# baudm/parseq

Hardware: NVIDIA H100
Metric: images/sec PARSeq-S 32x128 AR+1refine (higher is better)
Workload: dtype bf16

## Files before the change

### include/parseq_b200.h

```cpp
#ifndef PARSEQ_B200_H_
#define PARSEQ_B200_H_

#include <stdint.h>

#ifdef __cplusplus
extern "C" {
#endif

typedef struct parseq_engine parseq_engine;
typedef void* parseq_stream_t;

typedef enum parseq_status {
  PARSEQ_OK = 0,
  PARSEQ_ERR_INVALID_ARG = -1,
  PARSEQ_ERR_UNSUPPORTED = -2,
  PARSEQ_ERR_CUDA = -3,
  PARSEQ_ERR_STATE = -4,
  PARSEQ_ERR_NO_DEVICE = -5
} parseq_status;

typedef struct parseq_config {
  int32_t img_h, img_w;
  int32_t patch_h, patch_w;
  int32_t embed_dim;
// ... 65 lines not shown
int64_t parseq_kernel_launches(const parseq_engine* e);
int parseq_bench_tma_stream(void* buf, int64_t bytes, int cluster, int ctas, int nboxes, int nslot, int mode, void* sink,
                            parseq_stream_t stream);
int64_t parseq_debug_int(parseq_engine* e, const char* name);
int parseq_set_option(parseq_engine* e, const char* name, int64_t value);
int parseq_get_timing(parseq_engine* e, int category, double* ms, double* flops, int64_t* count);
int parseq_get_ar_profile(parseq_engine* e, uint64_t* out512);
const char* parseq_last_error(void);
const char* parseq_version(void);

int parseq_gemm_bf16(const void* A, int64_t lda, const void* W, int64_t ldw, const float* bias,
                     int M, int N, int K, int mode, float alpha, const float* resid, int64_t ldr,
                     int resid_mod, void* out, int64_t ldo, parseq_stream_t stream);
int parseq_gemm_ln_bf16(const void* A, int64_t lda, const void* W, int64_t ldw, const float* bias,
                        int M, int D, int K, float* x_inout, const float* gamma, const float* beta,
                        float eps, void* xn_bf16, parseq_stream_t stream);
int parseq_mlp_ln_bf16(const void* xn, const void* W1, const float* b1, const void* W2, const float* b2,
                       int M, int D, float* x_inout, const float* gamma, const float* beta, float eps,
                       void* xn_out_bf16, parseq_stream_t stream);
int parseq_layernorm_bf16(const float* x, const float* gamma, const float* beta, float eps, int M,
                          int D, void* y_bf16, float* y_f32_or_null, parseq_stream_t stream);
int parseq_enc_attention(const void* qkv_bf16, int B, int T, int D, int heads, void* out_bf16,
                         parseq_stream_t stream);

#ifdef __cplusplus
}
#endif
#endif
```

### parseq_b200/build.py

```python
from __future__ import annotations

import os
import shutil
import subprocess

PKG = os.path.dirname(os.path.abspath(__file__))
CSRC = os.path.join(PKG, "csrc")
LIB_DIR = os.path.join(PKG, "lib")
LIB_PATH = os.path.join(LIB_DIR, "libparseq_b200.so")
SOURCES = ["engine.cu"]
HEADERS = ["ptx.cuh", "gemm.cuh", "kernels.cuh", "dec_ar.cuh", "dec_ar2.cuh", "gemm_ln.cuh", "mlp_ln.cuh", "attn_wgmma.cuh", "crops.cuh", os.path.join("..", "..", "include", "parseq_b200.h")]

NVCC_FLAGS = [
    "-gencode", "arch=compute_90a,code=sm_90a", "-lineinfo", "-O3", "-std=c++17",
    "-Xcompiler", "-fPIC", "-shared",
]


def _nvcc() -> str:
    for cand in (os.environ.get("NVCC"), shutil.which("nvcc"), "/usr/local/cuda/bin/nvcc"):
        if cand and os.path.exists(cand):
            return cand
    raise RuntimeError("nvcc not found")


def needs_build() -> bool:
    if not os.path.exists(LIB_PATH):
        return True
    t = os.path.getmtime(LIB_PATH)
    deps = [os.path.join(CSRC, s) for s in SOURCES + HEADERS]
    return any(os.path.getmtime(d) > t for d in deps)


def build(force: bool = False, verbose: bool = False) -> str:
# ... 26 lines not shown
```

### parseq_b200/csrc/engine.cu

```cuda
#include <cuda.h>
#include <cuda_runtime.h>

#include <cmath>
#include <cstdio>
#include <cstdlib>
#include <cstring>
#include <map>
#include <mutex>
#include <set>
#include <string>
#include <type_traits>
#include <vector>

#include "../../include/parseq_b200.h"
#include "gemm.cuh"
#include "kernels.cuh"
#include "dec_ar.cuh"
#include "dec_ar2.cuh"
#include "gemm_ln.cuh"
#include "mlp_ln.cuh"
#include "attn_wgmma.cuh"
#include "crops.cuh"

namespace {

constexpr int kMaxHeadClasses = 16384;
constexpr int kMaxLabelLength = 63;

thread_local std::string g_last_error;

int fail(int code, const std::string& msg) {
  g_last_error = msg;
  return code;
}
#define PQ_CUDA(expr)                                                                              \
  do {                                                                                             \
    cudaError_t _e = (expr);                                                                       \
    if (_e != cudaSuccess)                                                                         \
      return fail(PARSEQ_ERR_CUDA, std::string(#expr) + " -> " + cudaGetErrorString(_e));          \
  } while (0)
#define PQ_TRY(expr)                 \
  do {                               \
    int _r = (expr);                 \
    if (_r != PARSEQ_OK) return _r;  \
// ... 187 lines not shown
}
template <int D, int MT, int CS, bool WIDE, int IDP>
int ar2_attr() {
  PQ_TRY(set_smem(ar2_kernel<D, MT, CS, false, WIDE, IDP>(), pq::dec_ar2_smem_bytes<D, MT, CS, IDP>()));
  if constexpr (MT == 1 && CS == 8 && D / 64 <= CS)
    PQ_TRY(set_smem(ar2_kernel<D, MT, CS, true, WIDE, IDP>(), pq::dec_ar2_smem_bytes<D, MT, CS, IDP>()));
  return PARSEQ_OK;
}
template <bool WIDE, int IDP>
int ar2_set_attributes() {
  PQ_TRY((ar2_attr<192, 1, 8, WIDE, IDP>())); PQ_TRY((ar2_attr<192, 2, 8, WIDE, IDP>())); PQ_TRY((ar2_attr<384, 1, 8, WIDE, IDP>()));
  PQ_TRY((ar2_attr<384, 2, 8, WIDE, IDP>())); PQ_TRY((ar2_attr<768, 1, 8, WIDE, IDP>()));
  PQ_TRY((ar2_attr<192, 1, 6, WIDE, IDP>())); PQ_TRY((ar2_attr<192, 2, 6, WIDE, IDP>())); PQ_TRY((ar2_attr<384, 1, 6, WIDE, IDP>()));
  PQ_TRY((ar2_attr<384, 2, 6, WIDE, IDP>())); PQ_TRY((ar2_attr<768, 1, 6, WIDE, IDP>()));
  return PARSEQ_OK;
}

template <int D, int MODE>
int gemm_ln_attr() { return set_smem(pq::gemm_ln_fused_kernel<D, MODE>, pq::GemmLnCfg<D, MODE>::kSmemBytes); }
template <int D, int CG>
int mlp_ln_attr() { return set_smem(pq::mlp_ln_fused_kernel<D, CG>, pq::MlpLnCfg<D, CG>::kSmemBytes); }
template <int NK>
int attn_wgmma_attr() { return set_smem(pq::enc_attention_wgmma_kernel<NK>, pq::atw_smem_bytes<NK>()); }
template <int EPI, int STORE>
int gemm_attr() { return set_smem(pq::gemm_bf16_wgmma_kernel<EPI, STORE>, pq::GemmCfg::smem_bytes<STORE != pq::ST_REG>()); }
constexpr int kTmaBenchSmem = 12 * pq::A2_SLOT + 1024 + 256;

int init_kernel_attributes() {
  PQ_TRY(set_smem(pq::dec_ar_kernel<192, 1>, pq::dec_ar_smem_bytes<192>()));
  PQ_TRY(set_smem(pq::dec_ar_kernel<192, 2>, pq::dec_ar_smem_bytes<192>()));
  PQ_TRY(set_smem(pq::dec_ar_kernel<384, 1>, pq::dec_ar_smem_bytes<384>()));
  PQ_TRY(set_smem(pq::dec_ar_kernel<384, 2>, pq::dec_ar_smem_bytes<384>()));
  PQ_TRY(set_smem(pq::dec_ar_kernel<768, 1>, pq::dec_ar_smem_bytes<768>()));
  PQ_TRY(set_smem(pq::dec_ar_kernel<768, 2>, pq::dec_ar_smem_bytes<768>()));
  PQ_TRY((ar2_set_attributes<false, 32>()));
  PQ_TRY((ar2_set_attributes<true, 32>()));
  PQ_TRY((ar2_set_attributes<false, 64>()));
  PQ_TRY((ar2_set_attributes<true, 64>()));
  PQ_TRY(set_smem(pq::dec_ln_head_argmax_kernel<192>, 120 * 1024));
  PQ_TRY(set_smem(pq::dec_ln_head_argmax_kernel<384>, 160 * 1024));
  PQ_TRY(set_smem(pq::dec_ln_head_argmax_kernel<768>, 226 * 1024));
  PQ_TRY((gemm_ln_attr<192, 0>())); PQ_TRY((gemm_ln_attr<384, 0>())); PQ_TRY((gemm_ln_attr<192, 1>()));
  PQ_TRY((gemm_ln_attr<384, 1>())); PQ_TRY((gemm_ln_attr<384, 2>()));
  PQ_TRY((mlp_ln_attr<192, 1>())); PQ_TRY((mlp_ln_attr<384, 1>())); PQ_TRY((mlp_ln_attr<192, 2>())); PQ_TRY((mlp_ln_attr<384, 2>()));
  PQ_TRY((attn_wgmma_attr<128>())); PQ_TRY((attn_wgmma_attr<256>()));
  PQ_TRY((gemm_attr<pq::EPI_F32, pq::ST_REG>()));
  PQ_TRY((gemm_attr<pq::EPI_F32_RESID, pq::ST_REG>()));
  PQ_TRY((gemm_attr<pq::EPI_BF16, pq::ST_REG>()));
  PQ_TRY((gemm_attr<pq::EPI_BF16, pq::ST_TMA_2D>()));
  PQ_TRY((gemm_attr<pq::EPI_BF16, pq::ST_TMA_3D>()));
  PQ_TRY((gemm_attr<pq::EPI_GELU_BF16, pq::ST_REG>()));
  PQ_TRY((gemm_attr<pq::EPI_GELU_BF16, pq::ST_TMA_2D>()));
  PQ_TRY(set_smem(pq::tma_stream_bench_kernel, kTmaBenchSmem));
  int dev = 0, optin = 0;
  PQ_CUDA(cudaGetDevice(&dev));
  PQ_CUDA(cudaDeviceGetAttribute(&optin, cudaDevAttrMaxSharedMemoryPerBlockOptin, dev));
  PQ_TRY(set_smem(pq::crop_resize_bicubic_kernel, static_cast<size_t>(optin)));
  return PARSEQ_OK;
}

int ensure_kernel_attributes() {
  static std::mutex mu;
  static std::set<int> done;
  int dev = 0;
  PQ_CUDA(cudaGetDevice(&dev));
  std::lock_guard<std::mutex> lock(mu);
  if (done.count(dev) != 0) return PARSEQ_OK;
  PQ_TRY(init_kernel_attributes());
// ... 133 lines not shown
    case 192: return launch_k(lo, pq::layernorm_kernel<192>, dim3(grid), dim3(256), 0, st, x, g, b, eps, M, yb, y32, add, add_mod, xw);
    case 384: return launch_k(lo, pq::layernorm_kernel<384>, dim3(grid), dim3(256), 0, st, x, g, b, eps, M, yb, y32, add, add_mod, xw);
    case 768: return launch_k(lo, pq::layernorm_kernel<768>, dim3(grid), dim3(256), 0, st, x, g, b, eps, M, yb, y32, add, add_mod, xw);
    default: return fail(PARSEQ_ERR_UNSUPPORTED, "layernorm: embed_dim must be 192, 384 or 768");
  }
}

int enc_attention_launch(const LaunchOpts& lo, const void* qkv, int B, int T, int D, int heads, void* out, cudaStream_t st) {
  if (D != heads * pq::ATT_DH) return fail(PARSEQ_ERR_UNSUPPORTED, "encoder attention kernels cover head_dim=64");
  if (lo.attn_impl == 1 && T <= 256) {
    const dim3 grid(static_cast<unsigned>(B * heads), static_cast<unsigned>((T + 127) / 128));
    const __nv_bfloat16* q = reinterpret_cast<const __nv_bfloat16*>(qkv);
    __nv_bfloat16* o = reinterpret_cast<__nv_bfloat16*>(out);
    if (T <= 128)
      return launch_k(lo, pq::enc_attention_wgmma_kernel<128>, grid, dim3(pq::ATW_THREADS), pq::atw_smem_bytes<128>(), st, q, o, T, D, heads);
    return launch_k(lo, pq::enc_attention_wgmma_kernel<256>, grid, dim3(pq::ATW_THREADS), pq::atw_smem_bytes<256>(), st, q, o, T, D, heads);
  }
  if (T != pq::ATT_T) {
    return launch_k(lo, pq::enc_attention_any_kernel, dim3(B * heads, (T + pq::ATT_T - 1) / pq::ATT_T), dim3(256), 0, st,
                    reinterpret_cast<const __nv_bfloat16*>(qkv), reinterpret_cast<__nv_bfloat16*>(out), T, D, heads);
  }
  return launch_k(lo, pq::enc_attention_kernel, dim3(B * heads), dim3(256), 0, st,
                  reinterpret_cast<const __nv_bfloat16*>(qkv), reinterpret_cast<__nv_bfloat16*>(out), D, heads);
}

struct Slot {
  std::string key;
  std::string pub;
  long long numel;
  bool bf16;
  void* dev;
  bool set;
};

}

struct parseq_engine {
  parseq_config cfg;
  int D, T, Kp, Me, Md, L, V, C, gh, gw, dh_dec;
  int ids_ld = 32;
  int arch = 0, Tp = 0;
  std::map<std::string, int> pub_index;
  float* vt_rows = nullptr;
  int chunk;
  std::vector<Slot> slots;
  std::map<std::string, int> index;
// ... 237 lines not shown
  }
  if (e->arch == 0) {
    PQ_TRY(gemm(e, e->a_pe, e->Kp, e->w("encoder.patch_embed.proj.weight"), e->Kp,
                e->wf("encoder.patch_embed.proj.bias"), M, D, e->Kp, pq::EPI_F32, 1.0f, e->wf("encoder.pos_embed"), D, T,
                e->x, D, st));
  } else {
    float* tmp = reinterpret_cast<float*>(e->hid);
    PQ_TRY(gemm(e, e->a_pe, e->Kp, e->w("encoder.patch_embed.proj.weight"), e->Kp,
                e->wf("encoder.patch_embed.proj.bias"), B * e->Tp, D, e->Kp, pq::EPI_F32, 1.0f,
                e->wf("encoder.pos_embed") + D, D, e->Tp, tmp, D, st));
    TimedScope ts(e, st, CAT_MISC, 0.0);
    const long long total = 1ll * M * (D / 4);
    const int grid = static_cast<int>(std::min<long long>((total + 255) / 256, 132ll * 16));
    PQ_TRY(launch_k(e->lo, pq::cls_assemble_kernel, dim3(grid), dim3(256), 0, st, reinterpret_cast<const float4*>(tmp),
                    reinterpret_cast<const float4*>(e->wf("encoder.cls_token")),
                    reinterpret_cast<const float4*>(e->wf("encoder.pos_embed")), reinterpret_cast<float4*>(e->x), B, e->Tp,
                    D / 4));
  }
  const int Mr = (regime_batch > B ? regime_batch : B) * T;
  const bool big = (Mr + pq::GEMM_BLOCK_M - 1) / pq::GEMM_BLOCK_M >= 2 * e->lo.sm_count || (e->fuse_ln & 4);
  const bool fuse_proj = (e->fuse_ln & 1) && gemm_ln_supported(D) && big;
  const bool fuse_fc2 = (e->fuse_ln & 2) && gemm_ln_supported(D) && big;
  const bool fuse_mlp = e->fuse_mlp && fuse_fc2 && e->Me == 4 * D;
  bool final_done = false;
  for (int i = 0; i < e->cfg.enc_depth; ++i) {
    const std::string p = "encoder.blocks." + std::to_string(i) + ".";
    const bool last = (i == e->cfg.enc_depth - 1);
    if (!(fuse_fc2 && i > 0)) PQ_TRY(layernorm(e, e->x, p + "norm1", 1e-6f, M, e->xn, nullptr, st));
    PQ_TRY(gemm(e, e->xn, D, e->w(p + "attn.qkv.weight"), D, e->wf(p + "attn.qkv.bias"), M, 3 * D, D, pq::EPI_BF16,
                1.0f, nullptr, 0, 0, e->qkv, 3 * D, st));
    {
      TimedScope ts(e, st, CAT_ENC_ATTN, 4.0 * B * T * T * D);
      PQ_TRY(enc_attention_launch(e->lo, e->qkv, B, T, D, e->cfg.enc_num_heads, e->att, st));
    }
    if (fuse_proj) {
      PQ_TRY(gemm_ln(e, e->att, D, p + "attn.proj", M, D, e->x, p + "norm2", 1e-6f, e->xn, st));
    } else {
      PQ_TRY(gemm(e, e->att, D, e->w(p + "attn.proj.weight"), D, e->wf(p + "attn.proj.bias"), M, D, D, pq::EPI_F32, 1.0f,
                  e->x, D, 0, e->x, D, st));
      PQ_TRY(layernorm(e, e->x, p + "norm2", 1e-6f, M, e->xn, nullptr, st));
    }
    if (fuse_mlp && (!last || (final_norm && memory32 == nullptr))) {
      if (!last) {
        PQ_TRY(mlp_ln(e, e->xn, p, M, e->x, "encoder.blocks." + std::to_string(i + 1) + ".norm1", 1e-6f, e->xn, st));
      } else {
        PQ_TRY(mlp_ln(e, e->xn, p, M, e->x, "encoder.norm", 1e-6f, mem_out, st));
        final_done = true;
      }
      continue;
    }
    PQ_TRY(gemm(e, e->xn, D, e->w(p + "mlp.fc1.weight"), D, e->wf(p + "mlp.fc1.bias"), M, e->Me, D, pq::EPI_GELU_BF16,
                1.0f, nullptr, 0, 0, e->hid, e->Me, st));
    if (fuse_fc2 && !last) {
      PQ_TRY(gemm_ln(e, e->hid, e->Me, p + "mlp.fc2", M, e->Me, e->x, "encoder.blocks." + std::to_string(i + 1) + ".norm1",
// ... 1346 lines not shown
}
int parseq_gemm_ln_bf16(const void* A, int64_t lda, const void* W, int64_t ldw, const float* bias, int M, int D, int K,
                         float* x_inout, const float* gamma, const float* beta, float eps, void* xn_bf16,
                         parseq_stream_t stream) {
  PQ_TRY(ensure_kernel_attributes());
  return gemm_ln_launch(g_default_opts, A, lda, W, ldw, bias, M, D, K, x_inout, gamma, beta, eps, xn_bf16, reinterpret_cast<cudaStream_t>(stream));
}
int parseq_mlp_ln_bf16(const void* xn, const void* W1, const float* b1, const void* W2, const float* b2, int M, int D,
                       float* x_inout, const float* gamma, const float* beta, float eps, void* xn_out_bf16, parseq_stream_t stream) {
  PQ_TRY(ensure_kernel_attributes());
  return mlp_ln_launch(g_default_opts, xn, W1, b1, W2, b2, M, D, x_inout, gamma, beta, eps, xn_out_bf16,
                       reinterpret_cast<cudaStream_t>(stream));
}
int parseq_layernorm_bf16(const float* x, const float* gamma, const float* beta, float eps, int M, int D, void* y_bf16,
                          float* y_f32_or_null, parseq_stream_t stream) {
  PQ_TRY(ensure_kernel_attributes());
  return layernorm_launch(g_default_opts, x, gamma, beta, eps, M, D, y_bf16, y_f32_or_null, reinterpret_cast<cudaStream_t>(stream));
}
int parseq_enc_attention(const void* qkv_bf16, int B, int T, int D, int heads, void* out_bf16, parseq_stream_t stream) {
  PQ_TRY(ensure_kernel_attributes());
  PQ_TRY(ensure_sm_count(g_default_opts));
  return enc_attention_launch(g_default_opts, qkv_bf16, B, T, D, heads, out_bf16, reinterpret_cast<cudaStream_t>(stream));
}

}
```

### parseq_b200/csrc/kernels.cuh

```cuda
#pragma once
#include "ptx.cuh"

namespace pq {

__global__ void im2col_patch_kernel(const float* __restrict__ img, __nv_bfloat16* __restrict__ out, int B, int H,
                                    int W, int ph, int pw, int gh, int gw) {
  grid_dep_launch();
  grid_dep_wait();
  const long long total = static_cast<long long>(B) * gh * gw * 3 * ph;
  const int Kp = 3 * ph * pw;
  for (long long i = blockIdx.x * static_cast<long long>(blockDim.x) + threadIdx.x; i < total;
       i += static_cast<long long>(gridDim.x) * blockDim.x) {
    long long t = i;
    const int c = static_cast<int>(t % gw); t /= gw;
    const int ch = static_cast<int>(t % 3); t /= 3;
    const int dy = static_cast<int>(t % ph); t /= ph;
    const int r = static_cast<int>(t % gh); t /= gh;
    const int b = static_cast<int>(t);
    const float* src = img + ((static_cast<long long>(b) * 3 + ch) * H + (r * ph + dy)) * W + c * pw;
    __nv_bfloat16* dst = out + (static_cast<long long>(b) * gh * gw + r * gw + c) * Kp + ch * ph * pw + dy * pw;
    if (pw == 8 && ((reinterpret_cast<uintptr_t>(src) & 15u) == 0) && ((reinterpret_cast<uintptr_t>(dst) & 15u) == 0)) {
      const float4 a = __ldg(reinterpret_cast<const float4*>(src));
      const float4 d = __ldg(reinterpret_cast<const float4*>(src) + 1);
      uint4 q;
// ... 72 lines not shown
    q += a * a + b * b;
  }
#pragma unroll
  for (int o = 16; o > 0; o >>= 1) q += __shfl_xor_sync(0xffffffffu, q, o);
  const float rstd = 1.0f / sqrtf(q * (1.0f / D) + eps);
  const float2* g2 = reinterpret_cast<const float2*>(gamma);
  const float2* b2 = reinterpret_cast<const float2*>(beta);
  uint32_t* yr = reinterpret_cast<uint32_t*>(y + static_cast<long long>(row) * D);
#pragma unroll
  for (int i = 0; i < NV; ++i) {
    const float2 g = __ldg(g2 + i * 32 + lane), b = __ldg(b2 + i * 32 + lane);
    const float o0 = (v[i].x - mean) * rstd * g.x + b.x;
    const float o1 = (v[i].y - mean) * rstd * g.y + b.y;
    yr[i * 32 + lane] = pack_bf16(o0, o1);
    if (y32 != nullptr) reinterpret_cast<float2*>(y32 + static_cast<long long>(row) * D)[i * 32 + lane] = make_float2(o0, o1);
  }
}

constexpr int ATT_T = 128;
constexpr int ATT_DH = 64;
__device__ __forceinline__ uint32_t att_swz(int r, int c) {
  return static_cast<uint32_t>(r * ATT_DH + ((((c >> 3) ^ (r & 7)) << 3) | (c & 7)));
}
__global__ void __launch_bounds__(256, 2) enc_attention_kernel(const __nv_bfloat16* __restrict__ qkv,
                                                            __nv_bfloat16* __restrict__ out, int D, int heads) {
  grid_dep_launch();
  grid_dep_wait();
  __shared__ __align__(128) __nv_bfloat16 sQ[ATT_T * ATT_DH];
  __shared__ __align__(128) __nv_bfloat16 sK[ATT_T * ATT_DH];
  __shared__ __align__(128) __nv_bfloat16 sV[ATT_T * ATT_DH];
  const int b = blockIdx.x / heads, h = blockIdx.x % heads;
  const int tid = threadIdx.x, warp = tid >> 5, lane = tid & 31;
  const long long ld = 3ll * D;
  const __nv_bfloat16* base = qkv + static_cast<long long>(b) * ATT_T * ld + h * ATT_DH;
  for (int i = tid; i < 3 * ATT_T * 8; i += 256) {
    const int m = i / (ATT_T * 8);
    const int r = (i / 8) % ATT_T;
    const int ck = i % 8;
    const __nv_bfloat16* src = base + static_cast<long long>(r) * ld + m * D + ck * 8;
    __nv_bfloat16* dstm = (m == 0) ? sQ : (m == 1) ? sK : sV;
    cp_async_16(smem_u32(dstm + att_swz(r, ck * 8)), src);
  }
  cp_async_wait_all();
  __syncthreads();

  const int r0 = warp * 16;
  uint32_t qf[4][4];
#pragma unroll
  for (int kt = 0; kt < 4; ++kt) {
    const int row = r0 + (lane & 7) + ((lane >> 3) & 1) * 8;
    const int col = kt * 16 + (lane >> 4) * 8;
    ldmatrix_x4(smem_u32(sQ + att_swz(row, col)), qf[kt][0], qf[kt][1], qf[kt][2], qf[kt][3]);
  }
  float sacc[16][4];
#pragma unroll
  for (int nt = 0; nt < 16; ++nt) { sacc[nt][0] = sacc[nt][1] = sacc[nt][2] = sacc[nt][3] = 0.f; }
#pragma unroll
  for (int kt = 0; kt < 4; ++kt) {
#pragma unroll
    for (int np = 0; np < 8; ++np) {
      const int key = np * 16 + (lane & 7) + (lane >> 4) * 8;
      const int col = kt * 16 + ((lane >> 3) & 1) * 8;
      uint32_t b0, b1, b2, b3;
      ldmatrix_x4(smem_u32(sK + att_swz(key, col)), b0, b1, b2, b3);
      mma_bf16_16816(sacc[2 * np], qf[kt][0], qf[kt][1], qf[kt][2], qf[kt][3], b0, b1);
      mma_bf16_16816(sacc[2 * np + 1], qf[kt][0], qf[kt][1], qf[kt][2], qf[kt][3], b2, b3);
    }
  }
  float mx0 = -INFINITY, mx1 = -INFINITY;
#pragma unroll
  for (int nt = 0; nt < 16; ++nt) {
    mx0 = fmaxf(mx0, fmaxf(sacc[nt][0], sacc[nt][1]));
    mx1 = fmaxf(mx1, fmaxf(sacc[nt][2], sacc[nt][3]));
  }
  mx0 = fmaxf(mx0, __shfl_xor_sync(0xffffffffu, mx0, 1));
  mx0 = fmaxf(mx0, __shfl_xor_sync(0xffffffffu, mx0, 2));
  mx1 = fmaxf(mx1, __shfl_xor_sync(0xffffffffu, mx1, 1));
  mx1 = fmaxf(mx1, __shfl_xor_sync(0xffffffffu, mx1, 2));
  constexpr float kScaleLog2 = 0.125f * 1.4426950408889634f;
  float sum0 = 0.f, sum1 = 0.f;
#pragma unroll
  for (int nt = 0; nt < 16; ++nt) {
    sacc[nt][0] = exp2f((sacc[nt][0] - mx0) * kScaleLog2);
    sacc[nt][1] = exp2f((sacc[nt][1] - mx0) * kScaleLog2);
    sacc[nt][2] = exp2f((sacc[nt][2] - mx1) * kScaleLog2);
    sacc[nt][3] = exp2f((sacc[nt][3] - mx1) * kScaleLog2);
    sum0 += sacc[nt][0] + sacc[nt][1];
    sum1 += sacc[nt][2] + sacc[nt][3];
  }
  sum0 += __shfl_xor_sync(0xffffffffu, sum0, 1);
  sum0 += __shfl_xor_sync(0xffffffffu, sum0, 2);
  sum1 += __shfl_xor_sync(0xffffffffu, sum1, 1);
  sum1 += __shfl_xor_sync(0xffffffffu, sum1, 2);
  float oacc[8][4];
#pragma unroll
  for (int nt = 0; nt < 8; ++nt) { oacc[nt][0] = oacc[nt][1] = oacc[nt][2] = oacc[nt][3] = 0.f; }
#pragma unroll
  for (int kk = 0; kk < 8; ++kk) {
    const uint32_t a0 = pack_bf16(sacc[2 * kk][0], sacc[2 * kk][1]);
    const uint32_t a1 = pack_bf16(sacc[2 * kk][2], sacc[2 * kk][3]);
    const uint32_t a2 = pack_bf16(sacc[2 * kk + 1][0], sacc[2 * kk + 1][1]);
    const uint32_t a3 = pack_bf16(sacc[2 * kk + 1][2], sacc[2 * kk + 1][3]);
#pragma unroll
    for (int np = 0; np < 4; ++np) {
      const int key = kk * 16 + (lane & 7) + ((lane >> 3) & 1) * 8;
      const int col = np * 16 + (lane >> 4) * 8;
      uint32_t b0, b1, b2, b3;
      ldmatrix_x4_trans(smem_u32(sV + att_swz(key, col)), b0, b1, b2, b3);
      mma_bf16_16816(oacc[2 * np], a0, a1, a2, a3, b0, b1);
      mma_bf16_16816(oacc[2 * np + 1], a0, a1, a2, a3, b2, b3);
    }
  }
  const float inv0 = 1.0f / sum0, inv1 = 1.0f / sum1;
  const int g = lane >> 2, t = lane & 3;
  __syncwarp();
#pragma unroll
  for (int nt = 0; nt < 8; ++nt) {
    const int col = nt * 8 + 2 * t;
    *reinterpret_cast<uint32_t*>(sQ + att_swz(r0 + g, col)) = pack_bf16(oacc[nt][0] * inv0, oacc[nt][1] * inv0);
    *reinterpret_cast<uint32_t*>(sQ + att_swz(r0 + g + 8, col)) = pack_bf16(oacc[nt][2] * inv1, oacc[nt][3] * inv1);
  }
  __syncwarp();
  __nv_bfloat16* obase = out + static_cast<long long>(b) * ATT_T * D + h * ATT_DH;
#pragma unroll
  for (int i = 0; i < 4; ++i) {
    const int idx = i * 32 + lane;
    const int r = r0 + (idx >> 3), ck = idx & 7;
    const uint4 val = *reinterpret_cast<const uint4*>(sQ + att_swz(r, ck * 8));
    *reinterpret_cast<uint4*>(obase + static_cast<long long>(r) * D + ck * 8) = val;
  }
}

__global__ void __launch_bounds__(256, 2) enc_attention_any_kernel(const __nv_bfloat16* __restrict__ qkv,
                                                                   __nv_bfloat16* __restrict__ out, int T, int D,
                                                                   int heads) {
  grid_dep_launch();
  grid_dep_wait();
  __shared__ __align__(128) __nv_bfloat16 sQ[ATT_T * ATT_DH];
  __shared__ __align__(128) __nv_bfloat16 sK[ATT_T * ATT_DH];
  __shared__ __align__(128) __nv_bfloat16 sV[ATT_T * ATT_DH];
  const int b = blockIdx.x / heads, h = blockIdx.x % heads;
  const int q0 = blockIdx.y * ATT_T;
  const int nkb = (T + ATT_T - 1) / ATT_T;
  const int tid = threadIdx.x, warp = tid >> 5, lane = tid & 31;
  const long long ld = 3ll * D;
  const __nv_bfloat16* base = qkv + static_cast<long long>(b) * T * ld + h * ATT_DH;
  auto load_tile = [&](__nv_bfloat16* dst, int mat, int row0, int nrows) {
    for (int i = tid; i < nrows * 8; i += 256) {
      const int r = i >> 3, ck = i & 7;
      int row = row0 + r;
      if (row >= T) row = T - 1;
      cp_async_16(smem_u32(dst + att_swz(r, ck * 8)), base + static_cast<long long>(row) * ld + mat * D + ck * 8);
    }
// ... 658 lines not shown
```

### parseq_b200/engine.py

```python
from __future__ import annotations

import ctypes as C
import os
from typing import Dict, Optional

from .build import LIB_PATH

_lib = None


class ParseqConfigC(C.Structure):
    _fields_ = [(n, C.c_int32) for n in (
        "img_h", "img_w", "patch_h", "patch_w", "embed_dim", "enc_num_heads", "enc_mlp_ratio", "enc_depth",
        "dec_num_heads", "dec_mlp_ratio", "dec_depth", "max_label_length", "num_tokens", "max_batch", "device", "arch")]


class ForwardArgsC(C.Structure):
    _fields_ = [("batch", C.c_int32), ("max_length", C.c_int32), ("decode_ar", C.c_int32),
                ("refine_iters", C.c_int32), ("forced_ids", C.c_void_p), ("forced_refine", C.c_void_p)]


class CropsC(C.Structure):
    _fields_ = [("data", C.c_void_p), ("data_bytes", C.c_int64), ("offsets", C.c_void_p), ("sizes", C.c_void_p),
                ("rotation", C.c_int32)]


EXPORTS = [
    "parseq_create", "parseq_destroy", "parseq_set_weight", "parseq_num_weights", "parseq_weight_key",
    "parseq_finalize", "parseq_forward", "parseq_forward_host", "parseq_forward_u8", "parseq_forward_host_u8",
    "parseq_resize_crops", "parseq_forward_crops", "parseq_forward_host_crops",
    "parseq_postprocess", "parseq_encode", "parseq_decode", "parseq_decode_ex", "parseq_head", "parseq_text_embed", "parseq_kernel_launches", "parseq_debug_int", "parseq_bench_tma_stream",
    "parseq_set_option", "parseq_get_timing", "parseq_get_ar_profile", "parseq_last_error", "parseq_version", "parseq_gemm_bf16", "parseq_gemm_ln_bf16", "parseq_mlp_ln_bf16", "parseq_layernorm_bf16",
    "parseq_enc_attention",
]


def load_library(path: Optional[str] = None):
    global _lib
    if _lib is not None and path is None:
        return _lib
    p = path or os.environ.get("PARSEQ_B200_LIB", LIB_PATH)
    if not os.path.exists(p):
        raise RuntimeError(f"{p} not found: build it with `python -m parseq_b200.build` "
                           "(there is no CPU / PyTorch fallback)")
    lib = C.CDLL(p)
    lib.parseq_last_error.restype = C.c_char_p
    lib.parseq_version.restype = C.c_char_p
    lib.parseq_weight_key.restype = C.c_char_p
    lib.parseq_weight_key.argtypes = [C.c_void_p, C.c_int, C.POINTER(C.c_int64)]
    lib.parseq_bench_tma_stream.argtypes = [C.c_void_p, C.c_int64, C.c_int, C.c_int, C.c_int, C.c_int, C.c_int, C.c_void_p, C.c_void_p]
    lib.parseq_debug_int.restype = C.c_int64
    lib.parseq_debug_int.argtypes = [C.c_void_p, C.c_char_p]
    lib.parseq_kernel_launches.restype = C.c_int64
    lib.parseq_kernel_launches.argtypes = [C.c_void_p]
    lib.parseq_create.argtypes = [C.POINTER(ParseqConfigC), C.POINTER(C.c_void_p)]
    lib.parseq_destroy.argtypes = [C.c_void_p]
# ... 12 lines not shown
    lib.parseq_forward_host_crops.argtypes = lib.parseq_forward_crops.argtypes
    lib.parseq_postprocess.argtypes = [C.c_void_p, C.c_int32, C.c_int32, C.c_int32, C.c_int32, C.c_void_p, C.c_void_p,
                                       C.c_void_p, C.c_void_p]
    lib.parseq_encode.argtypes = [C.c_void_p, C.c_int32, C.c_void_p, C.c_void_p, C.c_void_p]
    lib.parseq_decode.argtypes = [C.c_void_p, C.c_int32, C.c_int32, C.c_int32, C.c_void_p, C.c_void_p, C.c_void_p, C.c_void_p,
                                  C.c_void_p, C.c_void_p, C.c_void_p]
    lib.parseq_decode_ex.argtypes = [C.c_void_p, C.c_int32, C.c_int32, C.c_int32, C.c_void_p, C.c_void_p, C.c_void_p, C.c_void_p,
                                     C.c_void_p, C.c_void_p, C.c_void_p, C.c_void_p]
    lib.parseq_head.argtypes = [C.c_void_p, C.c_int32, C.c_void_p, C.c_void_p, C.c_void_p]
    lib.parseq_text_embed.argtypes = [C.c_void_p, C.c_int32, C.c_void_p, C.c_void_p, C.c_void_p]
    lib.parseq_set_option.argtypes = [C.c_void_p, C.c_char_p, C.c_int64]
    lib.parseq_get_timing.argtypes = [C.c_void_p, C.c_int, C.POINTER(C.c_double), C.POINTER(C.c_double),
                                      C.POINTER(C.c_int64)]
    lib.parseq_gemm_bf16.argtypes = [C.c_void_p, C.c_int64, C.c_void_p, C.c_int64, C.c_void_p, C.c_int, C.c_int,
                                     C.c_int, C.c_int, C.c_float, C.c_void_p, C.c_int64, C.c_int, C.c_void_p,
                                     C.c_int64, C.c_void_p]
    lib.parseq_gemm_ln_bf16.argtypes = [C.c_void_p, C.c_int64, C.c_void_p, C.c_int64, C.c_void_p, C.c_int, C.c_int, C.c_int,
                                        C.c_void_p, C.c_void_p, C.c_void_p, C.c_float, C.c_void_p, C.c_void_p]
    lib.parseq_mlp_ln_bf16.argtypes = [C.c_void_p, C.c_void_p, C.c_void_p, C.c_void_p, C.c_void_p, C.c_int, C.c_int, C.c_void_p,
                                       C.c_void_p, C.c_void_p, C.c_float, C.c_void_p, C.c_void_p]
    lib.parseq_layernorm_bf16.argtypes = [C.c_void_p, C.c_void_p, C.c_void_p, C.c_float, C.c_int, C.c_int,
                                          C.c_void_p, C.c_void_p, C.c_void_p]
    lib.parseq_enc_attention.argtypes = [C.c_void_p, C.c_int, C.c_int, C.c_int, C.c_int, C.c_void_p, C.c_void_p]
    if path is None:
        _lib = lib
    return lib


class EngineError(RuntimeError):
    pass


def check(lib, rc: int):
    if rc != 0:
        raise EngineError(f"parseq_b200 error {rc}: {lib.parseq_last_error().decode()}")


class Engine:

    def __init__(self, cfg, device: int = 0, max_batch: int = 0):
        self.lib = load_library()
        self.cfg = cfg
        c = ParseqConfigC(cfg.img_size[0], cfg.img_size[1], cfg.patch_size[0], cfg.patch_size[1], cfg.embed_dim,
                          cfg.enc_num_heads, cfg.enc_mlp_ratio, cfg.enc_depth, cfg.dec_num_heads, cfg.dec_mlp_ratio,
                          cfg.dec_depth, cfg.max_label_length, cfg.num_tokens, max_batch, device,
                          1 if getattr(cfg, "arch", "parseq") == "vitstr" else 0)
# ... 118 lines not shown
```

Before: 38900.

## Fuse encoder QKV projection GEMM with attention in a persistent warp-specialized kernel

Adds a persistent kernel that, for each (batch, head) item, computes the Q/K/V projection for a 128-token tile with TMA-fed wgmma and writes the results straight into swizzled shared memory. It then runs the existing 128x128 attention tile on that data, so the QKV activation never round-trips through global memory and one launch is removed per layer. The attention body is factored into a shared device function. In exchange, the activation tile is re-read once per head, and occupancy is one 384-thread CTA per SM with a producer warp group.

```diff
diff --git a/include/parseq_b200.h b/include/parseq_b200.h
--- a/include/parseq_b200.h
+++ b/include/parseq_b200.h
@@ -111,6 +111,8 @@
                           int D, void* y_bf16, float* y_f32_or_null, parseq_stream_t stream);
 int parseq_enc_attention(const void* qkv_bf16, int B, int T, int D, int heads, void* out_bf16,
                          parseq_stream_t stream);
+int parseq_qkv_attention_bf16(const void* xn_bf16, const void* W_qkv, const float* b_qkv, int B, int T, int D,
+                              int heads, void* out_bf16, parseq_stream_t stream);
 
 #ifdef __cplusplus
 }
diff --git a/parseq_b200/build.py b/parseq_b200/build.py
--- a/parseq_b200/build.py
+++ b/parseq_b200/build.py
@@ -9,7 +9,7 @@
 LIB_DIR = os.path.join(PKG, "lib")
 LIB_PATH = os.path.join(LIB_DIR, "libparseq_b200.so")
 SOURCES = ["engine.cu"]
-HEADERS = ["ptx.cuh", "gemm.cuh", "kernels.cuh", "dec_ar.cuh", "dec_ar2.cuh", "gemm_ln.cuh", "mlp_ln.cuh", "attn_wgmma.cuh", "crops.cuh", os.path.join("..", "..", "include", "parseq_b200.h")]
+HEADERS = ["ptx.cuh", "gemm.cuh", "kernels.cuh", "dec_ar.cuh", "dec_ar2.cuh", "gemm_ln.cuh", "mlp_ln.cuh", "attn_wgmma.cuh", "qkv_attn.cuh", "crops.cuh", os.path.join("..", "..", "include", "parseq_b200.h")]
 
 NVCC_FLAGS = [
     "-gencode", "arch=compute_90a,code=sm_90a", "-lineinfo", "-O3", "-std=c++17",
diff --git a/parseq_b200/csrc/engine.cu b/parseq_b200/csrc/engine.cu
--- a/parseq_b200/csrc/engine.cu
+++ b/parseq_b200/csrc/engine.cu
@@ -20,6 +20,7 @@
 #include "gemm_ln.cuh"
 #include "mlp_ln.cuh"
 #include "attn_wgmma.cuh"
+#include "qkv_attn.cuh"
 #include "crops.cuh"
 
 namespace {
@@ -253,6 +254,8 @@
 int mlp_ln_attr() { return set_smem(pq::mlp_ln_fused_kernel<D, CG>, pq::MlpLnCfg<D, CG>::kSmemBytes); }
 template <int NK>
 int attn_wgmma_attr() { return set_smem(pq::enc_attention_wgmma_kernel<NK>, pq::atw_smem_bytes<NK>()); }
+template <int D>
+int qkv_attn_attr() { return set_smem(pq::enc_qkv_attn_kernel<D>, pq::QkvAttnCfg::kSmemBytes); }
 template <int EPI, int STORE>
 int gemm_attr() { return set_smem(pq::gemm_bf16_wgmma_kernel<EPI, STORE>, pq::GemmCfg::smem_bytes<STORE != pq::ST_REG>()); }
 constexpr int kTmaBenchSmem = 12 * pq::A2_SLOT + 1024 + 256;
@@ -275,6 +278,7 @@
   PQ_TRY((gemm_ln_attr<384, 1>())); PQ_TRY((gemm_ln_attr<384, 2>()));
   PQ_TRY((mlp_ln_attr<192, 1>())); PQ_TRY((mlp_ln_attr<384, 1>())); PQ_TRY((mlp_ln_attr<192, 2>())); PQ_TRY((mlp_ln_attr<384, 2>()));
   PQ_TRY((attn_wgmma_attr<128>())); PQ_TRY((attn_wgmma_attr<256>()));
+  PQ_TRY((qkv_attn_attr<192>())); PQ_TRY((qkv_attn_attr<384>()));
   PQ_TRY((gemm_attr<pq::EPI_F32, pq::ST_REG>()));
   PQ_TRY((gemm_attr<pq::EPI_F32_RESID, pq::ST_REG>()));
   PQ_TRY((gemm_attr<pq::EPI_BF16, pq::ST_REG>()));
@@ -454,6 +458,25 @@
   }
   return launch_k(lo, pq::enc_attention_kernel, dim3(B * heads), dim3(256), 0, st,
                   reinterpret_cast<const __nv_bfloat16*>(qkv), reinterpret_cast<__nv_bfloat16*>(out), D, heads);
+}
+
+bool qkv_attn_supported(int T, int D, int heads) { return T == pq::ATT_T && D == heads * pq::ATT_DH && (D == 192 || D == 384); }
+int qkv_attn_launch(LaunchOpts& lo, const void* xn, const void* W, const float* bias, int B, int T, int D, int heads, void* out,
+                    cudaStream_t st) {
+  if (B <= 0) return fail(PARSEQ_ERR_INVALID_ARG, "qkv_attn: empty batch");
+  if (!qkv_attn_supported(T, D, heads))
+    return fail(PARSEQ_ERR_UNSUPPORTED, "qkv_attn: T = 128, head_dim 64 and embed_dim 192 or 384 only");
+  if ((reinterpret_cast<uintptr_t>(out) & 15u) != 0) return fail(PARSEQ_ERR_INVALID_ARG, "qkv_attn: out must be 16-byte aligned");
+  PQ_TRY(ensure_sm_count(lo));
+  CUtensorMap tx, tw;
+  PQ_TRY(make_tmap(&tx, xn, 2, static_cast<long long>(B) * T, D, D, pq::GEMM_BLOCK_K, pq::ATT_T));
+  PQ_TRY(make_tmap(&tw, W, 2, 3 * D, D, D, pq::GEMM_BLOCK_K, pq::ATT_DH));
+  const int items = B * heads;
+  const dim3 grid(static_cast<unsigned>(items < lo.sm_count ? items : lo.sm_count));
+  __nv_bfloat16* o = reinterpret_cast<__nv_bfloat16*>(out);
+  if (D == 192)
+    return launch_k(lo, pq::enc_qkv_attn_kernel<192>, grid, dim3(pq::QA_THREADS), pq::QkvAttnCfg::kSmemBytes, st, tx, tw, bias, o, items);
+  return launch_k(lo, pq::enc_qkv_attn_kernel<384>, grid, dim3(pq::QA_THREADS), pq::QkvAttnCfg::kSmemBytes, st, tx, tw, bias, o, items);
 }
 
 struct Slot {
@@ -737,14 +760,19 @@
   const bool fuse_proj = (e->fuse_ln & 1) && gemm_ln_supported(D) && big;
   const bool fuse_fc2 = (e->fuse_ln & 2) && gemm_ln_supported(D) && big;
   const bool fuse_mlp = e->fuse_mlp && fuse_fc2 && e->Me == 4 * D;
+  const bool fuse_qkv_attn = e->lo.attn_impl == 0 && qkv_attn_supported(T, D, e->cfg.enc_num_heads);
   bool final_done = false;
   for (int i = 0; i < e->cfg.enc_depth; ++i) {
     const std::string p = "encoder.blocks." + std::to_string(i) + ".";
     const bool last = (i == e->cfg.enc_depth - 1);
     if (!(fuse_fc2 && i > 0)) PQ_TRY(layernorm(e, e->x, p + "norm1", 1e-6f, M, e->xn, nullptr, st));
-    PQ_TRY(gemm(e, e->xn, D, e->w(p + "attn.qkv.weight"), D, e->wf(p + "attn.qkv.bias"), M, 3 * D, D, pq::EPI_BF16,
-                1.0f, nullptr, 0, 0, e->qkv, 3 * D, st));
-    {
+    if (fuse_qkv_attn) {
+      TimedScope ts(e, st, CAT_ENC_GEMM, 2.0 * M * 3 * D * D + 4.0 * B * T * T * D);
+      PQ_TRY(qkv_attn_launch(e->lo, e->xn, e->w(p + "attn.qkv.weight"), e->wf(p + "attn.qkv.bias"), B, T, D,
+                             e->cfg.enc_num_heads, e->att, st));
+    } else {
+      PQ_TRY(gemm(e, e->xn, D, e->w(p + "attn.qkv.weight"), D, e->wf(p + "attn.qkv.bias"), M, 3 * D, D, pq::EPI_BF16,
+                  1.0f, nullptr, 0, 0, e->qkv, 3 * D, st));
       TimedScope ts(e, st, CAT_ENC_ATTN, 4.0 * B * T * T * D);
       PQ_TRY(enc_attention_launch(e->lo, e->qkv, B, T, D, e->cfg.enc_num_heads, e->att, st));
     }
@@ -2137,5 +2165,10 @@
   PQ_TRY(ensure_sm_count(g_default_opts));
   return enc_attention_launch(g_default_opts, qkv_bf16, B, T, D, heads, out_bf16, reinterpret_cast<cudaStream_t>(stream));
 }
-
-}
+int parseq_qkv_attention_bf16(const void* xn_bf16, const void* W_qkv, const float* b_qkv, int B, int T, int D, int heads,
+                              void* out_bf16, parseq_stream_t stream) {
+  PQ_TRY(ensure_kernel_attributes());
+  return qkv_attn_launch(g_default_opts, xn_bf16, W_qkv, b_qkv, B, T, D, heads, out_bf16, reinterpret_cast<cudaStream_t>(stream));
+}
+
+}
diff --git a/parseq_b200/csrc/kernels.cuh b/parseq_b200/csrc/kernels.cuh
--- a/parseq_b200/csrc/kernels.cuh
+++ b/parseq_b200/csrc/kernels.cuh
@@ -118,6 +118,94 @@
 __device__ __forceinline__ uint32_t att_swz(int r, int c) {
   return static_cast<uint32_t>(r * ATT_DH + ((((c >> 3) ^ (r & 7)) << 3) | (c & 7)));
 }
+__device__ __forceinline__ void att_tile_128(__nv_bfloat16* sQ, const __nv_bfloat16* sK, const __nv_bfloat16* sV,
+                                             __nv_bfloat16* __restrict__ obase, int D, int warp, int lane) {
+  const int r0 = warp * 16;
+  uint32_t qf[4][4];
+#pragma unroll
+  for (int kt = 0; kt < 4; ++kt) {
+    const int row = r0 + (lane & 7) + ((lane >> 3) & 1) * 8;
+    const int col = kt * 16 + (lane >> 4) * 8;
+    ldmatrix_x4(smem_u32(sQ + att_swz(row, col)), qf[kt][0], qf[kt][1], qf[kt][2], qf[kt][3]);
+  }
+  float sacc[16][4];
+#pragma unroll
+  for (int nt = 0; nt < 16; ++nt) { sacc[nt][0] = sacc[nt][1] = sacc[nt][2] = sacc[nt][3] = 0.f; }
+#pragma unroll
+  for (int kt = 0; kt < 4; ++kt) {
+#pragma unroll
+    for (int np = 0; np < 8; ++np) {
+      const int key = np * 16 + (lane & 7) + (lane >> 4) * 8;
+      const int col = kt * 16 + ((lane >> 3) & 1) * 8;
+      uint32_t b0, b1, b2, b3;
+      ldmatrix_x4(smem_u32(sK + att_swz(key, col)), b0, b1, b2, b3);
+      mma_bf16_16816(sacc[2 * np], qf[kt][0], qf[kt][1], qf[kt][2], qf[kt][3], b0, b1);
+      mma_bf16_16816(sacc[2 * np + 1], qf[kt][0], qf[kt][1], qf[kt][2], qf[kt][3], b2, b3);
+    }
+  }
+  float mx0 = -INFINITY, mx1 = -INFINITY;
+#pragma unroll
+  for (int nt = 0; nt < 16; ++nt) {
+    mx0 = fmaxf(mx0, fmaxf(sacc[nt][0], sacc[nt][1]));
+    mx1 = fmaxf(mx1, fmaxf(sacc[nt][2], sacc[nt][3]));
+  }
+  mx0 = fmaxf(mx0, __shfl_xor_sync(0xffffffffu, mx0, 1));
+  mx0 = fmaxf(mx0, __shfl_xor_sync(0xffffffffu, mx0, 2));
+  mx1 = fmaxf(mx1, __shfl_xor_sync(0xffffffffu, mx1, 1));
+  mx1 = fmaxf(mx1, __shfl_xor_sync(0xffffffffu, mx1, 2));
+  constexpr float kScaleLog2 = 0.125f * 1.4426950408889634f;
+  float sum0 = 0.f, sum1 = 0.f;
+#pragma unroll
+  for (int nt = 0; nt < 16; ++nt) {
+    sacc[nt][0] = exp2f((sacc[nt][0] - mx0) * kScaleLog2);
+    sacc[nt][1] = exp2f((sacc[nt][1] - mx0) * kScaleLog2);
+    sacc[nt][2] = exp2f((sacc[nt][2] - mx1) * kScaleLog2);
+    sacc[nt][3] = exp2f((sacc[nt][3] - mx1) * kScaleLog2);
+    sum0 += sacc[nt][0] + sacc[nt][1];
+    sum1 += sacc[nt][2] + sacc[nt][3];
+  }
+  sum0 += __shfl_xor_sync(0xffffffffu, sum0, 1);
+  sum0 += __shfl_xor_sync(0xffffffffu, sum0, 2);
+  sum1 += __shfl_xor_sync(0xffffffffu, sum1, 1);
+  sum1 += __shfl_xor_sync(0xffffffffu, sum1, 2);
+  float oacc[8][4];
+#pragma unroll
+  for (int nt = 0; nt < 8; ++nt) { oacc[nt][0] = oacc[nt][1] = oacc[nt][2] = oacc[nt][3] = 0.f; }
+#pragma unroll
+  for (int kk = 0; kk < 8; ++kk) {
+    const uint32_t a0 = pack_bf16(sacc[2 * kk][0], sacc[2 * kk][1]);
+    const uint32_t a1 = pack_bf16(sacc[2 * kk][2], sacc[2 * kk][3]);
+    const uint32_t a2 = pack_bf16(sacc[2 * kk + 1][0], sacc[2 * kk + 1][1]);
+    const uint32_t a3 = pack_bf16(sacc[2 * kk + 1][2], sacc[2 * kk + 1][3]);
+#pragma unroll
+    for (int np = 0; np < 4; ++np) {
+      const int key = kk * 16 + (lane & 7) + ((lane >> 3) & 1) * 8;
+      const int col = np * 16 + (lane >> 4) * 8;
+      uint32_t b0, b1, b2, b3;
+      ldmatrix_x4_trans(smem_u32(sV + att_swz(key, col)), b0, b1, b2, b3);
+      mma_bf16_16816(oacc[2 * np], a0, a1, a2, a3, b0, b1);
+      mma_bf16_16816(oacc[2 * np + 1], a0, a1, a2, a3, b2, b3);
+    }
+  }
+  const float inv0 = 1.0f / sum0, inv1 = 1.0f / sum1;
+  const int g = lane >> 2, t = lane & 3;
+  __syncwarp();
+#pragma unroll
+  for (int nt = 0; nt < 8; ++nt) {
+    const int col = nt * 8 + 2 * t;
+    *reinterpret_cast<uint32_t*>(sQ + att_swz(r0 + g, col)) = pack_bf16(oacc[nt][0] * inv0, oacc[nt][1] * inv0);
+    *reinterpret_cast<uint32_t*>(sQ + att_swz(r0 + g + 8, col)) = pack_bf16(oacc[nt][2] * inv1, oacc[nt][3] * inv1);
+  }
+  __syncwarp();
+#pragma unroll
+  for (int i = 0; i < 4; ++i) {
+    const int idx = i * 32 + lane;
+    const int r = r0 + (idx >> 3), ck = idx & 7;
+    const uint4 val = *reinterpret_cast<const uint4*>(sQ + att_swz(r, ck * 8));
+    *reinterpret_cast<uint4*>(obase + static_cast<long long>(r) * D + ck * 8) = val;
+  }
+}
+
 __global__ void __launch_bounds__(256, 2) enc_attention_kernel(const __nv_bfloat16* __restrict__ qkv,
                                                             __nv_bfloat16* __restrict__ out, int D, int heads) {
   grid_dep_launch();
@@ -139,92 +227,7 @@
   }
   cp_async_wait_all();
   __syncthreads();
-
-  const int r0 = warp * 16;
-  uint32_t qf[4][4];
-#pragma unroll
-  for (int kt = 0; kt < 4; ++kt) {
-    const int row = r0 + (lane & 7) + ((lane >> 3) & 1) * 8;
-    const int col = kt * 16 + (lane >> 4) * 8;
-    ldmatrix_x4(smem_u32(sQ + att_swz(row, col)), qf[kt][0], qf[kt][1], qf[kt][2], qf[kt][3]);
-  }
-  float sacc[16][4];
-#pragma unroll
-  for (int nt = 0; nt < 16; ++nt) { sacc[nt][0] = sacc[nt][1] = sacc[nt][2] = sacc[nt][3] = 0.f; }
-#pragma unroll
-  for (int kt = 0; kt < 4; ++kt) {
-#pragma unroll
-    for (int np = 0; np < 8; ++np) {
-      const int key = np * 16 + (lane & 7) + (lane >> 4) * 8;
-      const int col = kt * 16 + ((lane >> 3) & 1) * 8;
-      uint32_t b0, b1, b2, b3;
-      ldmatrix_x4(smem_u32(sK + att_swz(key, col)), b0, b1, b2, b3);
-      mma_bf16_16816(sacc[2 * np], qf[kt][0], qf[kt][1], qf[kt][2], qf[kt][3], b0, b1);
-      mma_bf16_16816(sacc[2 * np + 1], qf[kt][0], qf[kt][1], qf[kt][2], qf[kt][3], b2, b3);
-    }
-  }
-  float mx0 = -INFINITY, mx1 = -INFINITY;
-#pragma unroll
-  for (int nt = 0; nt < 16; ++nt) {
-    mx0 = fmaxf(mx0, fmaxf(sacc[nt][0], sacc[nt][1]));
-    mx1 = fmaxf(mx1, fmaxf(sacc[nt][2], sacc[nt][3]));
-  }
-  mx0 = fmaxf(mx0, __shfl_xor_sync(0xffffffffu, mx0, 1));
-  mx0 = fmaxf(mx0, __shfl_xor_sync(0xffffffffu, mx0, 2));
-  mx1 = fmaxf(mx1, __shfl_xor_sync(0xffffffffu, mx1, 1));
-  mx1 = fmaxf(mx1, __shfl_xor_sync(0xffffffffu, mx1, 2));
-  constexpr float kScaleLog2 = 0.125f * 1.4426950408889634f;
-  float sum0 = 0.f, sum1 = 0.f;
-#pragma unroll
-  for (int nt = 0; nt < 16; ++nt) {
-    sacc[nt][0] = exp2f((sacc[nt][0] - mx0) * kScaleLog2);
-    sacc[nt][1] = exp2f((sacc[nt][1] - mx0) * kScaleLog2);
-    sacc[nt][2] = exp2f((sacc[nt][2] - mx1) * kScaleLog2);
-    sacc[nt][3] = exp2f((sacc[nt][3] - mx1) * kScaleLog2);
-    sum0 += sacc[nt][0] + sacc[nt][1];
-    sum1 += sacc[nt][2] + sacc[nt][3];
-  }
-  sum0 += __shfl_xor_sync(0xffffffffu, sum0, 1);
-  sum0 += __shfl_xor_sync(0xffffffffu, sum0, 2);
-  sum1 += __shfl_xor_sync(0xffffffffu, sum1, 1);
-  sum1 += __shfl_xor_sync(0xffffffffu, sum1, 2);
-  float oacc[8][4];
-#pragma unroll
-  for (int nt = 0; nt < 8; ++nt) { oacc[nt][0] = oacc[nt][1] = oacc[nt][2] = oacc[nt][3] = 0.f; }
-#pragma unroll
-  for (int kk = 0; kk < 8; ++kk) {
-    const uint32_t a0 = pack_bf16(sacc[2 * kk][0], sacc[2 * kk][1]);
-    const uint32_t a1 = pack_bf16(sacc[2 * kk][2], sacc[2 * kk][3]);
-    const uint32_t a2 = pack_bf16(sacc[2 * kk + 1][0], sacc[2 * kk + 1][1]);
-    const uint32_t a3 = pack_bf16(sacc[2 * kk + 1][2], sacc[2 * kk + 1][3]);
-#pragma unroll
-    for (int np = 0; np < 4; ++np) {
-      const int key = kk * 16 + (lane & 7) + ((lane >> 3) & 1) * 8;
-      const int col = np * 16 + (lane >> 4) * 8;
-      uint32_t b0, b1, b2, b3;
-      ldmatrix_x4_trans(smem_u32(sV + att_swz(key, col)), b0, b1, b2, b3);
-      mma_bf16_16816(oacc[2 * np], a0, a1, a2, a3, b0, b1);
-      mma_bf16_16816(oacc[2 * np + 1], a0, a1, a2, a3, b2, b3);
-    }
-  }
-  const float inv0 = 1.0f / sum0, inv1 = 1.0f / sum1;
-  const int g = lane >> 2, t = lane & 3;
-  __syncwarp();
-#pragma unroll
-  for (int nt = 0; nt < 8; ++nt) {
-    const int col = nt * 8 + 2 * t;
-    *reinterpret_cast<uint32_t*>(sQ + att_swz(r0 + g, col)) = pack_bf16(oacc[nt][0] * inv0, oacc[nt][1] * inv0);
-    *reinterpret_cast<uint32_t*>(sQ + att_swz(r0 + g + 8, col)) = pack_bf16(oacc[nt][2] * inv1, oacc[nt][3] * inv1);
-  }
-  __syncwarp();
-  __nv_bfloat16* obase = out + static_cast<long long>(b) * ATT_T * D + h * ATT_DH;
-#pragma unroll
-  for (int i = 0; i < 4; ++i) {
-    const int idx = i * 32 + lane;
-    const int r = r0 + (idx >> 3), ck = idx & 7;
-    const uint4 val = *reinterpret_cast<const uint4*>(sQ + att_swz(r, ck * 8));
-    *reinterpret_cast<uint4*>(obase + static_cast<long long>(r) * D + ck * 8) = val;
-  }
+  att_tile_128(sQ, sK, sV, out + static_cast<long long>(b) * ATT_T * D + h * ATT_DH, D, warp, lane);
 }
 
 __global__ void __launch_bounds__(256, 2) enc_attention_any_kernel(const __nv_bfloat16* __restrict__ qkv,
diff --git a/parseq_b200/csrc/qkv_attn.cuh b/parseq_b200/csrc/qkv_attn.cuh
--- /dev/null
+++ b/parseq_b200/csrc/qkv_attn.cuh
@@ -0,0 +1,109 @@
+#pragma once
+#include "gemm.cuh"
+#include "kernels.cuh"
+
+namespace pq {
+
+constexpr int QA_THREADS = 384;
+
+struct QkvAttnCfg {
+  static constexpr int kABytes = ATT_T * GEMM_BLOCK_K * 2;
+  static constexpr int kWBoxBytes = ATT_DH * GEMM_BLOCK_K * 2;
+  static constexpr int kStageBytes = kABytes + 3 * kWBoxBytes;
+  static constexpr int kTileBytes = ATT_T * ATT_DH * 2;
+  static constexpr int kStages = 4;
+  static constexpr int kSmemBytes = kStages * kStageBytes + 3 * kTileBytes + 1024  + 256 ;
+};
+static_assert(QkvAttnCfg::kSmemBytes <= 232448, "shared memory");
+
+template <int D>
+__global__ void __launch_bounds__(QA_THREADS, 1)
+enc_qkv_attn_kernel(const __grid_constant__ CUtensorMap tmX, const __grid_constant__ CUtensorMap tmW,
+                    const float* __restrict__ bias, __nv_bfloat16* __restrict__ out, int num_items) {
+  static_assert(D == 192 || D == 384, "embed_dim");
+  using Cfg = QkvAttnCfg;
+  constexpr int kHeads = D / ATT_DH;
+  constexpr int kNumKb = D / GEMM_BLOCK_K;
+  extern __shared__ uint8_t smem_raw[];
+  const uint32_t raw_addr = smem_u32(smem_raw);
+  const uint32_t pad = ((raw_addr + 1023u) & ~1023u) - raw_addr;
+  uint8_t* smem = smem_raw + pad;
+  __nv_bfloat16* sQ = reinterpret_cast<__nv_bfloat16*>(smem + Cfg::kStages * Cfg::kStageBytes);
+  __nv_bfloat16* sK = sQ + ATT_T * ATT_DH;
+  __nv_bfloat16* sV = sK + ATT_T * ATT_DH;
+  uint64_t* full_bar = reinterpret_cast<uint64_t*>(sV + ATT_T * ATT_DH);
+  uint64_t* empty_bar = full_bar + Cfg::kStages;
+
+  const int n_local = (num_items - 1 - static_cast<int>(blockIdx.x)) / static_cast<int>(gridDim.x) + 1;
+
+  grid_dep_launch();
+  if (threadIdx.x == 0) {
+    prefetch_tmap(&tmX);
+    prefetch_tmap(&tmW);
+    for (int s = 0; s < Cfg::kStages; ++s) {
+      mbar_init(&full_bar[s], 1);
+      mbar_init(&empty_bar[s], 2);
+    }
+    fence_mbar_init();
+  }
+  __syncthreads();
+  grid_dep_wait();
+
+  if (threadIdx.x < 128) {
+    setmaxnreg_dec<40>();
+    if (threadIdx.x == 0) {
+      int stage = 0;
+      uint32_t phase = 0;
+      for (int j = 0; j < n_local; ++j) {
+        const int item = static_cast<int>(blockIdx.x) + j * static_cast<int>(gridDim.x);
+        const int m0 = (item / kHeads) * ATT_T, h = item % kHeads;
+        for (int kb = 0; kb < kNumKb; ++kb) {
+          mbar_wait_mma(&empty_bar[stage], phase ^ 1u);
+          uint8_t* sa = smem + stage * Cfg::kStageBytes;
+          mbar_expect_tx(&full_bar[stage], Cfg::kStageBytes);
+          tma_load_2d(sa, &tmX, &full_bar[stage], kb * GEMM_BLOCK_K, m0);
+#pragma unroll
+          for (int m = 0; m < 3; ++m)
+            tma_load_2d(sa + Cfg::kABytes + m * Cfg::kWBoxBytes, &tmW, &full_bar[stage], kb * GEMM_BLOCK_K,
+                        m * D + h * ATT_DH);
+          if (++stage == Cfg::kStages) { stage = 0; phase ^= 1u; }
+        }
+      }
+    }
+  } else {
+    setmaxnreg_inc<232>();
+    const int wg = (threadIdx.x >> 7) - 1;
+    const int lane = threadIdx.x & 31;
+    const int warp = (threadIdx.x >> 5) - 4;
+    const int r0 = 64 * wg + 16 * (warp & 3) + (lane >> 2);
+    int stage = 0;
+    uint32_t phase = 0;
+#pragma unroll 1
+    for (int j = 0; j < n_local; ++j) {
+      const int item = static_cast<int>(blockIdx.x) + j * static_cast<int>(gridDim.x);
+      const int b = item / kHeads, h = item % kHeads;
+      float acc[3 * ATT_DH / 2];
+#pragma unroll
+      for (int i = 0; i < 3 * ATT_DH / 2; ++i) acc[i] = 0.0f;
+      wg_mainloop<3 * ATT_DH, false>(acc, smem, Cfg::kStageBytes, wg * (Cfg::kABytes / 2), Cfg::kABytes, full_bar,
+                                     empty_bar, Cfg::kStages, kNumKb, stage, phase);
+      if (j > 0) named_bar_sync(1, 256);
+#pragma unroll
+      for (int i = 0; i < 3 * ATT_DH / 8; ++i) {
+        const int m = i / 8, c = (i % 8) * 8 + 2 * (lane & 3);
+        const int col = m * D + h * ATT_DH + c;
+        const float b0 = bias != nullptr ? __ldg(bias + col) : 0.0f;
+        const float b1 = bias != nullptr ? __ldg(bias + col + 1) : 0.0f;
+        __nv_bfloat16* dst = m == 0 ? sQ : m == 1 ? sK : sV;
+        *reinterpret_cast<uint32_t*>(dst + att_swz(r0, c)) =
+            pack_bf16(gemm_epi<EPI_BF16>(acc[4 * i], b0, 1.0f), gemm_epi<EPI_BF16>(acc[4 * i + 1], b1, 1.0f));
+        *reinterpret_cast<uint32_t*>(dst + att_swz(r0 + 8, c)) =
+            pack_bf16(gemm_epi<EPI_BF16>(acc[4 * i + 2], b0, 1.0f), gemm_epi<EPI_BF16>(acc[4 * i + 3], b1, 1.0f));
+      }
+      named_bar_sync(1, 256);
+      att_tile_128(sQ, sK, sV, out + static_cast<long long>(b) * ATT_T * D + h * ATT_DH, D, warp, lane);
+    }
+  }
+}
+
+}
diff --git a/parseq_b200/engine.py b/parseq_b200/engine.py
--- a/parseq_b200/engine.py
+++ b/parseq_b200/engine.py
@@ -31,7 +31,7 @@
     "parseq_resize_crops", "parseq_forward_crops", "parseq_forward_host_crops",
     "parseq_postprocess", "parseq_encode", "parseq_decode", "parseq_decode_ex", "parseq_head", "parseq_text_embed", "parseq_kernel_launches", "parseq_debug_int", "parseq_bench_tma_stream",
     "parseq_set_option", "parseq_get_timing", "parseq_get_ar_profile", "parseq_last_error", "parseq_version", "parseq_gemm_bf16", "parseq_gemm_ln_bf16", "parseq_mlp_ln_bf16", "parseq_layernorm_bf16",
-    "parseq_enc_attention",
+    "parseq_enc_attention", "parseq_qkv_attention_bf16",
 ]
 
 
@@ -90,6 +90,8 @@
     lib.parseq_layernorm_bf16.argtypes = [C.c_void_p, C.c_void_p, C.c_void_p, C.c_float, C.c_int, C.c_int,
                                           C.c_void_p, C.c_void_p, C.c_void_p]
     lib.parseq_enc_attention.argtypes = [C.c_void_p, C.c_int, C.c_int, C.c_int, C.c_int, C.c_void_p, C.c_void_p]
+    lib.parseq_qkv_attention_bf16.argtypes = [C.c_void_p, C.c_void_p, C.c_void_p, C.c_int, C.c_int, C.c_int, C.c_int,
+                                              C.c_void_p, C.c_void_p]
     if path is None:
         _lib = lib
     return lib
```

Result: faster. 41210, median of 6 (+6.0%).
